# tyb311/TCCT

Measured on AMD Instinct MI355X. Metric: OCT B-scans/sec fwd+bwd(+clip+AdamW), stc_tt bs=8 1x800x1100, higher is better.
Workload: dtype bf16; 1 GPU; stc_tt --los=di bs=8/GPU 1x800x1100 (net tensors 3x800x1104); global_batch=8, parallelism=dp1, ranks=1, grad_allreduce=none, slowest_step=66

## Files before the change

include/tcct_hip.h:

```cpp
#ifndef TCCT_HIP_H
#define TCCT_HIP_H
#include <stdint.h>
#ifdef __cplusplus
extern "C" {
#endif

typedef void* tcct_stream_t;

enum { TCCT_F32 = 0, TCCT_BF16 = 1 };
enum { TCCT_ACT_NONE = 0, TCCT_ACT_LRELU = 1, TCCT_ACT_HSWISH = 2, TCCT_ACT_GELU = 3, TCCT_ACT_SIGMOID = 4,
       TCCT_ACT_ABS = 5 };
enum { TCCT_CRIT_DICE = 0, TCCT_CRIT_DICE2 = 1, TCCT_CRIT_IOU = 2, TCCT_CRIT_MSE = 3 };

int tcct_version(void);
const char* tcct_last_error(void);
int tcct_set_outputs_prezeroed(int on);

int tcct_image_to_nhwc4(const float* img, void* out, int N, int Csrc, int H, int Wsrc, int Wdst, int dtype,
                        tcct_stream_t stream);
int tcct_u8_gather2d(const uint8_t* src, uint8_t* dst, int N, int SH, int SW, int C, int sy0, int sx0, int sh, int sw, int DH, int DW,
                     int dy0, int dx0, int dh, int dw, int flipy, int flipx, int mul, int div, int fill, tcct_stream_t stream);
int tcct_onehot_to_index(const int64_t* onehot, uint8_t* lab, int N, int C, int64_t HW, tcct_stream_t stream);
int tcct_labels_to_u8(const int64_t* lab, uint8_t* out, int N, int H, int Wsrc, int Wdst, tcct_stream_t stream);
int tcct_nhwc_to_nchw_f32(const void* x, float* y, int N, int64_t HW, int C, int dtype, tcct_stream_t stream);
// ... 97 lines not shown

int tcct_conv32_fwd_bnstats(const void* x, const void* wp, const float* bias, void* y, int N, int H, int W, int KH, int KW, int PH,
                            int PW, double* stats, int pre_act, tcct_stream_t stream);
int tcct_conv32_fwd_affine(const void* x, const void* wp, const float* bias, void* y, int N, int H, int W, int KH, int KW,
                           int PH, int PW, const float* ab, int pre_act, int post_act, tcct_stream_t stream);
int tcct_pw_fwd_affine(const void* x, const float* w, const float* bias, void* y, int64_t M, int K, int N, const float* ab,
                       int pre_act, int post_act, int out_dtype, tcct_stream_t stream);
int tcct_pw_fwd_affine_residual(const void* x, const float* w, const float* bias, const float* ab, const void* res, void* y, int64_t M, int K, int N,
                                tcct_stream_t stream);
int tcct_pw_fwd_cat2_affine(const void* x1, const void* x2, const float* w, const float* bias, const float* ab, int post_act, void* y, int64_t M, int K, int N,
                            tcct_stream_t stream);
int tcct_pw_fwd_xaff_affine_residual(const void* y_prev, const float* ab_prev, const float* w, const float* bias, const float* ab, const void* res, void* y,
                                     int64_t M, int K, int N, tcct_stream_t stream);
int tcct_conv32_fwd_add(const void* x, const void* wp, const float* bias, const void* res, void* y, int N, int H, int W, int KH, int KW,
                        int PH, int PW, tcct_stream_t stream);
int tcct_conv32_chain33(const void* x, const void* wp1, const float* bias1, void* mid, const void* wp2, const float* bias2, void* y,
                        const void* res, int N, int H, int W, double* stats, tcct_stream_t stream);
int tcct_conv32_pack_weights_sub(const float* w, void* wp, int KH, int KW, int transposed, int cin_total, int o_off, int i_off,
                                 tcct_stream_t stream);
int tcct_conv32_fwd_strided(const void* x, const void* wp, const float* bias, void* y, int N, int H, int W, int KH, int KW, int PH,
                            int PW, int xs, int xo, int ys, int yo, int accumulate, tcct_stream_t stream);
int tcct_conv32_fwd_strided_bnstats(const void* x, const void* wp, const float* bias, void* y, int N, int H, int W, int KH, int KW, int PH,
                                    int PW, int xs, int xo, int ys, int yo, int accumulate, double* stats, int pre_act, tcct_stream_t stream);
int tcct_conv32_fwd_strided_affine(const void* x, const void* wp, const float* bias, void* y, int N, int H, int W, int KH, int KW, int PH, int PW, int xs,
                                   int xo, int ys, int yo, const float* ab, int pre_act, int post_act, tcct_stream_t stream);
int64_t tcct_conv32_wgrad_mode(int mode);
int64_t tcct_conv32_fwd_mode(int mode);
int tcct_conv32_wgrad_strided(const void* x, const void* dy, float* dw, float* dbias, int N, int H, int W, int KH, int KW, int PH,
                              int PW, int xs, int xo, int ds, int dof, int cin_total, int o_off, int i_off, tcct_stream_t stream);
int tcct_conv32_wgrad(const void* x, const void* dy, float* dw, float* dbias, int N, int H, int W, int KH, int KW, int PH,
                      int PW, tcct_stream_t stream);
int tcct_conv32_bwd3x3(const void* x, const void* dy, const void* wp_t, const void* dskip, void* dx, float* dw, float* dbias, int N, int H,
                       int W, tcct_stream_t stream);

int tcct_pw_fwd(const void* x, const float* w, const float* bias, void* y, int64_t M, int K, int N, int transposed,
                int out_dtype, tcct_stream_t stream);
int tcct_pw_wgrad(const void* x, const void* dy, float* dw, float* dbias, int64_t M, int K, int N, tcct_stream_t stream);
int tcct_pw_bwd(const void* x, const void* dy, const float* w, const void* res, void* dx, float* dw, float* dbias, int64_t M, int K, int N,
                tcct_stream_t stream);
int tcct_pw_bwd_cat2(const void* x1, const void* x2, const void* dy, const float* w, void* dx1, void* dx2, float* dw, int64_t M, int K, int N,
                     tcct_stream_t stream);
int tcct_pw_bwd_residual2(const void* x, const void* dy, const float* w, const void* res, void* dx_sum, void* dx_plain, float* dw, float* dbias,
                          int64_t M, int K, int N, tcct_stream_t stream);
int64_t tcct_pw_bwd_bn_supported(int K, int N, int post, int red_post, int split);
int tcct_pw_bwd_bn(const void* x, const void* x2, const void* dz, const void* y, const float* coef, int post, const float* w, const void* res,
                   void* dx, void* dx2, float* dw, float* dbias, int64_t M, int K, int N, const void* y_prev, const float* ab_prev,
                   int red_post, double* sums_prev, tcct_stream_t stream);
int tcct_pw_bwd_bn_sums(const void* x, const void* x2, const void* dz, const void* y, const double* sums, int raw, const float* mean_rstd,
                        const float* ab, float* dgamma, float* dbeta, int post, const float* w, const void* res, void* dx, void* dx2, float* dw,
                        float* dbias, int64_t M, int K, int N, const void* y_prev, const float* ab_prev, int red_post, double* sums_prev,
                        tcct_stream_t stream);
int tcct_pw_wgrad_strided(const void* x, const void* dy, int64_t ldy, float* dw, float* dbias, int64_t M, int K, int N,
                          tcct_stream_t stream);
int tcct_pw_fwd_residual(const void* x, const float* w, const float* bias, const void* res, const float* scale, int64_t per_sample,
                         void* y, void* y_plain, int64_t M, int K, int N, tcct_stream_t stream);
int tcct_pw_fwd_bnstats_xaff(const void* y_prev, const float* ab_prev, const float* w, const float* bias, void* y, int64_t M, int K, int N, double* stats,
                             tcct_stream_t stream);
int tcct_pw_bwd_bn_sums_xaff(const void* y_prev, const float* ab_prev, const void* dz, const void* y, const double* sums, int raw, const float* mean_rstd,
                             const float* ab, float* dgamma, float* dbeta, const float* w, const void* res, void* dx, float* dw, float* dbias, int64_t M,
                             int K, int N, int red_post, double* sums_prev, tcct_stream_t stream);
int tcct_pw_fwd_gelu_residual(const void* x1, const float* w, const float* bias, const void* res, const float* scale, int64_t per_sample, void* y,
                              int64_t M, int K, int N, tcct_stream_t stream);
int tcct_pw_bwd_residual2_sum(const void* x, const void* dy_a, const void* dy_b, const float* w, const void* res, void* dx_sum, void* dx_plain, float* dw,
                              float* dbias, int64_t M, int K, int N, tcct_stream_t stream);
int tcct_pw_bwd_lnb(const void* x, const void* dy, const float* w, const void* t, const float* mean_rstd, const float* gamma, const void* res, void* dt,
                    float* dw, float* dbias, float* dgamma, float* dbeta, int64_t M, int K, int N, tcct_stream_t stream);
// ... 203 lines not shown
```

tcct_amd/csrc/conv_mfma.hip:

```cpp
#include "common.h"

typedef __attribute__((ext_vector_type(8))) __bf16 bf16x8;
typedef __attribute__((ext_vector_type(16))) float f32x16;

#define MB 256
#define OOB_OFF 0x80000000u

__global__ void k_pack_w32(const float* __restrict__ w, bf16* __restrict__ wp, int KH, int KW, int transposed, int ldi,
                           int o_off, int i_off) {
    int total = KH * KW * 32 * 32;
    for (int i = blockIdx.x * blockDim.x + threadIdx.x; i < total; i += gridDim.x * blockDim.x) {
        int ci = i & 31, co = (i >> 5) & 31, tap = i >> 10;
        int dy = tap / KW, dx = tap % KW;
        const float vt = w[(((int64_t)(o_off + ci) * ldi + i_off + co) * KH + (KH - 1 - dy)) * KW + (KW - 1 - dx)];
        const float vn = w[(((int64_t)(o_off + co) * ldi + i_off + ci) * KH + dy) * KW + dx];
        if (transposed == 2) { wp[i] = __float2bfloat16(vn); wp[total + i] = __float2bfloat16(vt); }
        else wp[i] = __float2bfloat16(transposed ? vt : vn);
    }
}
extern "C" int tcct_conv32_pack_weights(const float* w, void* wp, int KH, int KW, int transposed, tcct_stream_t stream) {
    int total = KH * KW * 1024;
    hipLaunchKernelGGL(k_pack_w32, dim3((total + MB - 1) / MB), dim3(MB), 0, (hipStream_t)stream, w, (bf16*)wp, KH, KW, transposed, 32, 0, 0);
    TCCT_LAUNCH_OK();
}
// ... 1812 lines not shown
            TCCT_LAUNCH_OK();
        }
    }
    constexpr bool line_on = true;
    if (line_on && g_wgrad_mode != 1 && (KH == 1 || KW == 1) && (TAPS == 13 || TAPS == 11 || TAPS == 9) && xs == 32 && ds == 32 && ldi == 32 && o_off == 0 && i_off == 0 &&
        xo == 0 && dof == 0) {
#define WL_LAUNCH(KK, V)                                                                                                     \
    do {                                                                                                                    \
        tcct_launch<k_conv32_wgrad_line<KK, V>, 80 * 1024>(dim3(grid), dim3(MB), (size_t)(8 * (64 + KK - 1) + 16) * 64 + 512 * 64, st, (const bf16*)x, (const bf16*)dy, \
                           dw, dbias, N, H, W, tilesH, tilesW, (int)nt);                                                    \
    } while (0)
        if (TAPS == 13) { if (vert) WL_LAUNCH(13, true); else WL_LAUNCH(13, false); }
        else if (TAPS == 11) { if (vert) WL_LAUNCH(11, true); else WL_LAUNCH(11, false); }
        else { if (vert) WL_LAUNCH(9, true); else WL_LAUNCH(9, false); }
#undef WL_LAUNCH
        TCCT_LAUNCH_OK();
    }
    const int TG = TAPS > 10 ? 4 : (TAPS > 5 ? 2 : 1);
    const int tpw = (TAPS + TG - 1) / TG;
    TCCT_CHECK(TAPS <= 16, "conv32_wgrad: %d taps unsupported", TAPS);
    TCCT_CHECK(LH * LW * 4 <= MAXL * MB, "conv32_wgrad: %dx%d tile image exceeds the staging slots", KH, KW);
#define WG_LAUNCH(TPW, V, Q)                                                                                                 \
    do {                                                                                                                    \
        tcct_launch<k_conv32_wgrad<TPW, V, Q>, 80 * 1024>(dim3(grid), dim3(MB), lds, st, (const bf16*)x, (const bf16*)dy, dw, dbias, N, H, W, KH, \
                           KW, PH, PW, TG, tilesH, tilesW, (int)nt, xs, xo, ds, dof, ldi, o_off, i_off);                                                        \
    } while (0)
    if (sq) WG_LAUNCH(5, false, true);
    else if (tpw <= 4) { if (vert) WG_LAUNCH(4, true, false); else WG_LAUNCH(4, false, false); }
    else { if (vert) WG_LAUNCH(5, true, false); else WG_LAUNCH(5, false, false); }
#undef WG_LAUNCH
    TCCT_LAUNCH_OK();
}

#define BWD_T 512
template <int DUMMY>
__global__ void __launch_bounds__(BWD_T, 1)
k_conv32_bwd33(const bf16* __restrict__ x, const bf16* __restrict__ dy, const bf16* __restrict__ wp, const bf16* __restrict__ dskip,
               bf16* __restrict__ dx, float* __restrict__ dw, float* __restrict__ dbias, int N, int H, int W, int tilesH, int tilesW,
               int ntiles) {
    constexpr int TH = 16, TW = 32, LH = 18, LW = 34, NPIX = LH * LW, SLOTS = (NPIX * 4 + BWD_T - 1) / BWD_T;
    extern __shared__ __attribute__((aligned(16))) unsigned char smem[];
    unsigned char* sW = smem;
    unsigned char* sXl = smem + 9 * 2048;
    unsigned char* sDp = sXl + NPIX * 64;
    unsigned char* sS = sDp + NPIX * IPS;
    const int tid = threadIdx.x, lane = tid & 63, wave = tid >> 6;
    const int r = lane & 31, hh = lane >> 5;
    for (int i = tid; i < 9 * 32 * 4; i += BWD_T) {
        int row = i >> 2, c4 = i & 3;
        uint4 v = reinterpret_cast<const uint4*>(wp)[i];
        *reinterpret_cast<uint4*>(sW + row * 64 + ((c4 ^ ((row >> 2) & 3)) << 4)) = v;
    }
    const int c = tid & 3;
    int s_rc[SLOTS];
#pragma unroll
    for (int j = 0; j < SLOTS; ++j) {
        int pl = (tid >> 2) + j * (BWD_T / 4);
        bool in = pl < NPIX;
        int lr = in ? pl / LW : 0x3fff, lc = in ? pl - (pl / LW) * LW : 0;
        s_rc[j] = (lr << 16) | lc;
    }
    const uint32_t img_bytes = (uint32_t)H * (uint32_t)W * 64u;
    u32x4 px[SLOTS], pd[SLOTS];
    auto prefetch = [&](int tile) {
        const int tw = tile % tilesW;
        const int t2 = tile / tilesW;
        const int th = t2 % tilesH;
        const int n = t2 / tilesH;
        const int hb = th * TH - 1, wb = tw * TW - 1;
        const __amdgpu_buffer_rsrc_t rx = __builtin_amdgcn_make_buffer_rsrc((void*)(x + (int64_t)n * H * W * 32), 0, img_bytes, 0x00020000);
        const __amdgpu_buffer_rsrc_t rd = __builtin_amdgcn_make_buffer_rsrc((void*)(dy + (int64_t)n * H * W * 32), 0, img_bytes, 0x00020000);
#pragma unroll
        for (int j = 0; j < SLOTS; ++j) {
            const int hi = hb + (s_rc[j] >> 16), wi = wb + (s_rc[j] & 0xffff);
            const bool ok = (unsigned)hi < (unsigned)H && (unsigned)wi < (unsigned)W;
            const uint32_t off = ok ? (uint32_t)((hi * W + wi) * 64 + c * 16) : OOB_OFF;
            px[j] = __builtin_amdgcn_raw_buffer_load_b128(rx, off, 0, 0);
            pd[j] = __builtin_amdgcn_raw_buffer_load_b128(rd, off, 0, 0);
        }
    };
    auto stage = [&]() {
#pragma unroll
        for (int j = 0; j < SLOTS; ++j) {
            const int lr = s_rc[j] >> 16, lc = s_rc[j] & 0xffff;
            if (lr != 0x3fff) {
                const int p = lr * LW + lc;
                *reinterpret_cast<u32x4*>(sXl + p * 64 + c * 16) = px[j];
                *reinterpret_cast<u32x4*>(sDp + p * IPS + c * 16) = pd[j];
            }
        }
    };
    const int wsw = (r >> 2) & 3;
    const unsigned char* wA0 = sW + r * 64 + ((hh ^ wsw) << 4);
    const unsigned char* wA1 = sW + r * 64 + (((2 + hh) ^ wsw) << 4);
    const int dwave = wave & 3;
    const unsigned char* xB[4];
#pragma unroll
    for (int t = 0; t < 4; ++t) xB[t] = sDp + ((dwave * 4 + t) * LW + r) * IPS + hh * 16;
    const int tg = (wave >> 1) & 1, wi = wave & 1;
    const int tap0 = tg * 5;
    int poff[5];
#pragma unroll
    for (int t = 0; t < 5; ++t) {
        const int tap = tap0 + t, ky = tap / 3, kx = tap - ky * 3;
        poff[t] = tap < 9 ? (ky * LW + kx) * 64 : 0;
    }
    f32x16 accw[5];
#pragma unroll
    for (int t = 0; t < 5; ++t)
#pragma unroll
        for (int k = 0; k < 16; ++k) accw[t][k] = 0.f;
    float bsum = 0.f;
    const int li = lane & 15, lq = li >> 2, lpp = li & 3, lg = lane >> 4;
    const unsigned char* lbX = sXl + (8 * (lg >> 1) + lq) * 64 + (16 * (lg & 1) + 4 * lpp) * 2;
    const unsigned char* lbD = sDp + (8 * (lg >> 1) + lq) * IPS + (16 * (lg & 1) + 4 * lpp) * 2;
    auto tr8 = [&](const unsigned char* p, int stride) {
        s16x4 lo = __builtin_amdgcn_ds_read_tr16_b64_v4i16((__attribute__((address_space(3))) s16x4*)p);
        s16x4 hi = __builtin_amdgcn_ds_read_tr16_b64_v4i16((__attribute__((address_space(3))) s16x4*)(p + 4 * stride));
        s16x8 v = __builtin_shufflevector(lo, hi, 0, 1, 2, 3, 4, 5, 6, 7);
        return __builtin_bit_cast(bf16x8, v);
    };

    int tile = blockIdx.x;
    if (tile < ntiles) {
        prefetch(tile);
        __syncthreads();
        stage();
        if (tile + (int)gridDim.x < ntiles) prefetch(tile + gridDim.x);
    }
    __syncthreads();
    for (; tile < ntiles; tile += gridDim.x) {
        const int tw = tile % tilesW;
        const int t2 = tile / tilesW;
        const int th = t2 % tilesH;
        const int n = t2 / tilesH;
        const int h0 = th * TH, w0 = tw * TW;
        f32x16* const acc = accw;
        if (wave < 4) {
#pragma unroll
            for (int t = 0; t < 4; ++t)
#pragma unroll
                for (int k = 0; k < 16; ++k) acc[t][k] = 0.f;
            struct Frag { bf16x8 a, b[4]; };
            auto load_stage = [&](Frag& f, int ky, int kx, int half) {
                f.a = *reinterpret_cast<const bf16x8*>((half ? wA1 : wA0) + (ky * 3 + kx) * 2048);
                const int po = (ky * LW + kx) * IPS + half * 32;
#pragma unroll
                for (int t = 0; t < 4; ++t) f.b[t] = *reinterpret_cast<const bf16x8*>(xB[t] + po);
            };
            Frag f[2];
            load_stage(f[0], 0, 0, 0);
#pragma unroll
            for (int k = 0; k < 18; ++k) {
                if (k + 1 < 18) load_stage(f[(k + 1) & 1], ((k + 1) >> 1) / 3, ((k + 1) >> 1) % 3, (k + 1) & 1);
                __builtin_amdgcn_sched_barrier(0);
#pragma unroll
                for (int t = 0; t < 4; ++t) acc[t] = __builtin_amdgcn_mfma_f32_32x32x16_bf16(f[k & 1].a, f[k & 1].b[t], acc[t], 0, 0, 0);
                __builtin_amdgcn_sched_barrier(0);
            }
        } else {
            struct WF { bf16x8 a, b[5]; };
            auto load_chunk = [&](WF& f, int ch) {
                const int a = ch >> 1, s16 = (ch & 1) * 16;
                f.a = tr8(lbD + ((a + 1) * LW + s16 + 1) * IPS, IPS);
                const unsigned char* pxb = lbX + (a * LW + s16) * 64;
#pragma unroll
                for (int t = 0; t < 5; ++t) f.b[t] = tr8(pxb + poff[t], 64);
            };
            auto mma_chunk = [&](const WF& f) {
                if (tg == 0) {
#pragma unroll
                    for (int j = 0; j < 4; ++j) bsum = dot2_ones(f.a, j, bsum);
                }
#pragma unroll
                for (int t = 0; t < 5; ++t)
                    if (tap0 + t < 9) accw[t] = __builtin_amdgcn_mfma_f32_32x32x16_bf16(f.a, f.b[t], accw[t], 0, 0, 0);
            };
            WF f0, f1;
            load_chunk(f0, wi);
            for (int ch = wi; ch < 32; ch += 4) {
                load_chunk(f1, ch + 2);
                __builtin_amdgcn_sched_barrier(0);
                mma_chunk(f0);
                __builtin_amdgcn_sched_barrier(0);
                if (ch + 4 < 32) load_chunk(f0, ch + 4);
                __builtin_amdgcn_sched_barrier(0);
                mma_chunk(f1);
                __builtin_amdgcn_sched_barrier(0);
            }
        }
        __syncthreads();
        if (tile + (int)gridDim.x < ntiles) stage();
        if (tile + 2 * (int)gridDim.x < ntiles) prefetch(tile + 2 * gridDim.x);
        if (wave < 4) {
            const __amdgpu_buffer_rsrc_t ws = __builtin_amdgcn_make_buffer_rsrc((void*)(dx + (int64_t)n * H * W * 32), 0, img_bytes, 0x00020000);
            const __amdgpu_buffer_rsrc_t rsk = __builtin_amdgcn_make_buffer_rsrc((void*)((dskip ? dskip : dx) + (int64_t)n * H * W * 32), 0, img_bytes, 0x00020000);
            unsigned char* sc = sS + dwave * 1024;
#pragma unroll
            for (int t = 0; t < 4; ++t) {
                const int a = dwave * 4 + t;
                uint2 o[4];
#pragma unroll
                for (int q = 0; q < 4; ++q) {
                    o[q].x = pack_bf16x2(acc[t][4 * q], acc[t][4 * q + 1]);
                    o[q].y = pack_bf16x2(acc[t][4 * q + 2], acc[t][4 * q + 3]);
                }
#pragma unroll
                for (int h2 = 0; h2 < 2; ++h2) {
                    if ((r >> 4) == h2) {
                        const int rr = r & 15, fsw = (rr >> 1) & 3;
#pragma unroll
                        for (int q = 0; q < 4; ++q) *reinterpret_cast<uint2*>(sc + rr * 64 + ((q ^ fsw) << 4) + hh * 8) = o[q];
                    }
                    wave_lds_fence();
                    const int p16 = lane >> 2, cch = lane & 3;
                    u32x4 ov = *reinterpret_cast<const u32x4*>(sc + p16 * 64 + ((cch ^ ((p16 >> 1) & 3)) << 4));
                    const int ho = h0 + a, wo = w0 + 16 * h2 + p16;
                    const uint32_t off = (ho < H && wo < W) ? (uint32_t)((ho * W + wo) * 64 + cch * 16) : OOB_OFF;
                    if (dskip) {
                        const u32x4 sv = __builtin_amdgcn_raw_buffer_load_b128(rsk, off, 0, 0);
#pragma unroll
                        for (int k = 0; k < 4; ++k)
                            ov[k] = pack_bf16x2(__uint_as_float(ov[k] << 16) + __uint_as_float(sv[k] << 16),
                                                __uint_as_float(ov[k] & 0xffff0000u) + __uint_as_float(sv[k] & 0xffff0000u));
                    }
                    __builtin_amdgcn_raw_buffer_store_b128(ov, ws, off, 0, 0);
                    wave_lds_fence();
                }
            }
        }
        __syncthreads();
    }
    __syncthreads();
    float* red = reinterpret_cast<float*>(sXl);
    for (int turn = 0; turn < 2; ++turn) {
        if (wave >= 4 && wi == turn) {
#pragma unroll
            for (int t = 0; t < 5; ++t) {
                const int tap = tap0 + t;
                if (tap < 9) {
#pragma unroll
                    for (int k = 0; k < 16; ++k) {
                        const int co = (k & 3) + 8 * (k >> 2) + 4 * hh;
                        float* dst = &red[tap * 1024 + co * 32 + r];
                        *dst = turn == 0 ? accw[t][k] : *dst + accw[t][k];
                    }
                }
            }
        }
        __syncthreads();
    }
    for (int i = tid; i < 9 * 1024; i += BWD_T) {
        const int tap = i % 9, cc = i / 9;
        atomicAdd(&dw[(int64_t)cc * 9 + tap], red[tap * 1024 + cc]);
    }
    if (dbias && wave >= 4 && tg == 0) {
        bsum += __shfl_xor(bsum, 32, 64);
        if (lane < 32) atomicAdd(&dbias[r], bsum);
    }
}

extern "C" int tcct_conv32_bwd3x3(const void* x, const void* dy, const void* wp_t, const void* dskip, void* dx, float* dw, float* dbias,
                                  int N, int H, int W, tcct_stream_t stream) {
    TCCT_CHECK((int64_t)H * W * 64 < (1LL << 31), "conv32_bwd3x3: image exceeds the 2 GiB buffer-descriptor range");
    TCCT_CHECK(dskip != dx, "conv32_bwd3x3: dskip must be a separate tensor");
    hipStream_t st = (hipStream_t)stream;
    if (!tcct_skip_zero_fill() && hipMemsetAsync(dw, 0, sizeof(float) * 9 * 1024, st) != hipSuccess) { tcct_set_error("conv32_bwd3x3: memset failed"); return -2; }
    if (dbias && !tcct_skip_zero_fill() && hipMemsetAsync(dbias, 0, sizeof(float) * 32, st) != hipSuccess) { tcct_set_error("conv32_bwd3x3: memset failed"); return -2; }
    const int tilesH = (H + 15) / 16, tilesW = (W + 31) / 32;
    const int64_t nt = (int64_t)N * tilesH * tilesW;
    TCCT_CHECK(nt > 0 && nt < (1LL << 31), "conv32_bwd3x3: bad tile count");
    const size_t lds = 9 * 2048 + (size_t)18 * 34 * 64 + (size_t)18 * 34 * IPS + 4096;
    const int grid = (int)(nt < 256 ? nt : 256);
    tcct_launch<k_conv32_bwd33<0>, 160 * 1024>(dim3(grid), dim3(BWD_T), lds, st, (const bf16*)x, (const bf16*)dy, (const bf16*)wp_t, (const bf16*)dskip,
                       (bf16*)dx, dw, dbias, N, H, W, tilesH, tilesW, (int)nt);
    TCCT_LAUNCH_OK();
}
```

tcct_amd/ops.py:

```python
import os
import weakref

import torch

from ._lib import lib, dtype_code, TcctError, launch_on, F32, BF16

ACT = {None: 0, 'none': 0, 'lrelu': 1, 'hswish': 2, 'gelu': 3, 'sigmoid': 4, 'abs': 5}


class _ZeroPool:

    def __init__(self):
        self.buf = None
        self.off = 0
        self.active = False
        self.frozen = False

    def begin(self, device, nbytes=8 << 20):
        if self.buf is None or self.buf.device != device or self.buf.numel() < nbytes:
            if self.frozen:
                raise TcctError('the zero pool cannot be re-allocated after a training step was captured into a hipGraph '
                                f'(pool on {self.buf.device}, step on {device})')
            self.buf = torch.empty(nbytes, device=device, dtype=torch.uint8)
        self.buf.zero_()
# ... 277 lines not shown
            and 32 <= Cin <= 256 and 32 <= Cout <= 256 and (Cin, Cout) != (32, 32) and stride == 1
            and 2 * padh == KH - 1 and 2 * padw == KW - 1 and 1 < KH * KW <= 13 and (KH == 1 or KW == 1 or (KH == 3 and KW == 3)))


def _conv_slabs_fwd_f32(x, w, bias, y, N, H, W, Cin, Cout, KH, KW, padh, padw, transposed):
    for oh in range(Cout // 32):
        for ih in range(Cin // 32):
            wp = torch.empty(KH * KW * 1024, device=x.device, dtype=torch.float32)
            if not transposed:
                lib.conv32f_pack_weights_sub(w, wp, KH, KW, 0, Cin, 32 * oh, 32 * ih)
            else:
                lib.conv32f_pack_weights_sub(w, wp, KH, KW, 1, Cout, 32 * ih, 32 * oh)
            b = bias[32 * oh:32 * oh + 32] if (bias is not None and ih == 0) else None
            lib.conv32f_fwd_strided(x, wp, b, y, N, H, W, KH, KW, padh, padw, Cin, 32 * ih, Cout, 32 * oh, 1 if ih > 0 else 0)


def _conv_slabs_fwd(x, w, bias, y, N, H, W, Cin, Cout, KH, KW, padh, padw, transposed, stats=None, stat_pre=0):
    wp = torch.empty(KH * KW * 1024, device=x.device, dtype=torch.bfloat16)
    for oh in range(Cout // 32):
        for ih in range(Cin // 32):
            if not transposed:
                lib.conv32_pack_weights_sub(w, wp, KH, KW, 0, Cin, 32 * oh, 32 * ih)
            else:
                lib.conv32_pack_weights_sub(w, wp, KH, KW, 1, Cout, 32 * ih, 32 * oh)
            b = bias[32 * oh:32 * oh + 32] if (bias is not None and ih == 0) else None
            if stats is not None and ih == Cin // 32 - 1:
                lib.conv32_fwd_strided_bnstats(x, wp, b, y, N, H, W, KH, KW, padh, padw, Cin, 32 * ih, Cout, 32 * oh, 1 if ih > 0 else 0, stats, stat_pre)
            else:
                lib.conv32_fwd_strided(x, wp, b, y, N, H, W, KH, KW, padh, padw, Cin, 32 * ih, Cout, 32 * oh, 1 if ih > 0 else 0)
            if ih + 1 < Cin // 32 or oh + 1 < Cout // 32:
                wp = torch.empty_like(wp)


FUSED_CONV_BWD = False
FUSED_PW_BWD = True


def _pw_bwd_ok(x, dy, Cin, Cin_w, Cout, KH, KW, stride, padh, padw):
    return (x.dtype == torch.bfloat16 and dy.dtype == torch.bfloat16 and KH == 1 and KW == 1 and stride == 1 and padh == 0 and padw == 0
            and Cin == Cin_w and Cin % 32 == 0 and Cout % 32 == 0 and 32 <= Cin <= 128 and 32 <= Cout <= 128
            and x.numel() * 2 < 2 ** 31 and dy.numel() * 2 < 2 ** 31)


def _pw_ok(in_dt, Cin, Cin_w, KH, KW, stride, padh, padw):
    return (in_dt == torch.bfloat16 and KH == 1 and KW == 1 and stride == 1 and padh == 0 and padw == 0 and Cin == Cin_w
            and Cin % 32 == 0)


class _Conv2d(_FastFunction):
    @staticmethod
    def forward(ctx, x, w, bias, stride, padh, padw, out_dtype, stats_box, fork=False):
        ctx.set_materialize_grads(False)
        _chk(x, w, bias)
        N, H, W, Cin = x.shape
        Cout, Cin_w, KH, KW = w.shape
        Ho = (H + 2 * padh - KH) // stride + 1
        Wo = (W + 2 * padw - KW) // stride + 1
        odt = out_dtype or x.dtype
        y = torch.empty((N, Ho, Wo, Cout), device=x.device, dtype=odt)
        mfma = _mfma32_ok(x.dtype, odt, Cin, Cin_w, Cout, KH, KW, stride, padh, padw)
        if _pw_ok(x.dtype, Cin, Cin_w, KH, KW, stride, padh, padw) and not mfma:
            if stats_box is not None and odt == torch.bfloat16 and Cout % 32 == 0 and Cout <= 160:
                sums = ZERO.get((2 * Cout,), torch.float64, x.device) if ZERO.active else torch.zeros(2 * Cout, device=x.device, dtype=torch.float64)
                lib.pw_fwd_bnstats(x, w, bias, y, N * H * W, Cin, Cout, sums, stats_box[0])
                stats_box[1] = sums
            else:
                lib.pw_fwd(x, w, bias, y, N * H * W, Cin, Cout, 0, dtype_code(odt))
# ... 28 lines not shown
            _conv_slabs_fwd_f32(x, w, bias, y, N, H, W, Cin, Cout, KH, KW, padh, padw, False)
        elif F32_PW[0] and _pwf_ok(x.dtype, odt, Cin, Cin_w, Cout, KH, KW, stride, padh, padw):
            lib.pwf_fwd(x, w, bias, y, N * H * W, Cin, Cout, 0)
        else:
            lib.conv2d_fwd(x, w, bias, y, N, H, W, Cin, Cin_w, Cout, KH, KW, stride, padh, padw, dtype_code(x.dtype),
                           dtype_code(odt))
        ctx.save_for_backward(x, w)
        ctx.cfg = (stride, padh, padw, bias is not None)
        wsrc = w if hasattr(w, '_grad_slot') or w._base is None else w._base
        ctx.params = (wsrc, bias)
        return (y, x.view_as(x)) if fork else y

    @staticmethod
    def backward(ctx, dy, dskip=None):
        x, w = ctx.saved_tensors
        stride, padh, padw, has_bias = ctx.cfg
        wsrc, bsrc = ctx.params
        if dy is None:
            return dskip, None, None, None, None, None, None, None, None
        dy = _c(dy)
        if dskip is not None:
            dskip = _as(dskip, x.dtype)
        N, H, W, Cin = x.shape
        Cout, Cin_w, KH, KW = w.shape
        dx = dw = db = None
        if (FUSED_PW_BWD and ctx.needs_input_grad[0] and ctx.needs_input_grad[1] and _pw_bwd_ok(x, dy, Cin, Cin_w, Cout, KH, KW, stride, padh, padw)
                and (dskip is None or dskip.shape == x.shape)):
            dx = torch.empty_like(x)
            dw = _grad_out(wsrc, tuple(w.shape))
            db = _grad_out(bsrc) if has_bias else None
            lib.pw_bwd(x, dy, w, dskip, dx, dw, db, N * H * W, Cin, Cout)
            return dx, _ret(dw, wsrc), _ret(db, bsrc), None, None, None, None, None, None
        if (FUSED_CONV_BWD and ctx.needs_input_grad[0] and ctx.needs_input_grad[1] and KH == 3 and KW == 3 and dy.dtype == torch.bfloat16
                and _mfma32_ok(x.dtype, dy.dtype, Cin, Cin_w, Cout, KH, KW, stride, padh, padw) and H * W * 64 < 2 ** 31):
            wp = getattr(ctx, 'wp_t', None)
            if wp is None:
                wp = torch.empty(9 * 1024, device=x.device, dtype=torch.bfloat16)
                lib.conv32_pack_weights(w, wp, 3, 3, 1)
            dx = torch.empty_like(x)
            dw = _grad_out(wsrc, tuple(w.shape))
            db = _grad_out(bsrc) if has_bias else None
            lib.conv32_bwd3x3(x, dy, wp, dskip, dx, dw, db, N, H, W)
            return dx, _ret(dw, wsrc), _ret(db, bsrc), None, None, None, None, None, None
        if ctx.needs_input_grad[0]:
            if stride != 1 or Cin != Cin_w:
                raise TcctError('conv2d dgrad: only stride-1 convs with unpadded channels need an input gradient')
            dx = torch.empty_like(x)
            if (_pw_ok(dy.dtype, Cout, Cout, KH, KW, stride, padh, padw) and x.dtype == torch.bfloat16
                    and not _mfma32_ok(dy.dtype, x.dtype, Cout, Cout, Cin, KH, KW, stride, padh, padw)):
                if dskip is not None and Cin % 32 == 0:
                    lib.pw_dgrad_residual(dy, w, dskip, dx, None, N * H * W, Cout, Cin)
                    dskip = None
                else:
                    lib.pw_fwd(dy, w, None, dx, N * H * W, Cout, Cin, 1, dtype_code(x.dtype))
            elif _mfma_slabs_ok(dy.dtype, x.dtype, Cout, Cout, Cin, KH, KW, stride, padh, padw):
                _conv_slabs_fwd(dy, w, None, dx, N, H, W, Cout, Cin, KH, KW, KH - 1 - padh, KW - 1 - padw, True)
            elif _mfma32_ok(dy.dtype, x.dtype, Cout, Cout, Cin, KH, KW, stride, padh, padw):
                wp = getattr(ctx, 'wp_t', None)
                if wp is None:
                    wp = torch.empty(KH * KW * 1024, device=x.device, dtype=torch.bfloat16)
                    lib.conv32_pack_weights(w, wp, KH, KW, 1)
                if dskip is not None:
                    lib.conv32_fwd_add(dy, wp, None, dskip, dx, N, H, W, KH, KW, KH - 1 - padh, KW - 1 - padw)
                    dskip = None
                else:
                    lib.conv32_fwd(dy, wp, None, dx, N, H, W, KH, KW, KH - 1 - padh, KW - 1 - padw)
            elif _mfma_slabs_f32_ok(dy.dtype, x.dtype, Cout, Cout, Cin, KH, KW, stride, padh, padw):
# ... 2785 lines not shown
```

Measured before the change: 420.5 B-scans/s.

## Stream fused 3x3 conv backward over row strips with LDS DMA ring and enable it

```diff
diff --git a/include/tcct_hip.h b/include/tcct_hip.h
--- a/include/tcct_hip.h
+++ b/include/tcct_hip.h
@@ -153,6 +153,8 @@
                       int PW, tcct_stream_t stream);
 int tcct_conv32_bwd3x3(const void* x, const void* dy, const void* wp_t, const void* dskip, void* dx, float* dw, float* dbias, int N, int H,
                        int W, tcct_stream_t stream);
+int64_t tcct_conv32_bwd_mode(int mode);
+int64_t tcct_conv32_bwd_streams(int N, int H, int W);
 
 int tcct_pw_fwd(const void* x, const float* w, const float* bias, void* y, int64_t M, int K, int N, int transposed,
                 int out_dtype, tcct_stream_t stream);
diff --git a/tcct_amd/csrc/conv_mfma.hip b/tcct_amd/csrc/conv_mfma.hip
--- a/tcct_amd/csrc/conv_mfma.hip
+++ b/tcct_amd/csrc/conv_mfma.hip
@@ -1868,247 +1868,294 @@
     TCCT_LAUNCH_OK();
 }
 
-#define BWD_T 512
-template <int DUMMY>
-__global__ void __launch_bounds__(BWD_T, 1)
-k_conv32_bwd33(const bf16* __restrict__ x, const bf16* __restrict__ dy, const bf16* __restrict__ wp, const bf16* __restrict__ dskip,
-               bf16* __restrict__ dx, float* __restrict__ dw, float* __restrict__ dbias, int N, int H, int W, int tilesH, int tilesW,
-               int ntiles) {
-    constexpr int TH = 16, TW = 32, LH = 18, LW = 34, NPIX = LH * LW, SLOTS = (NPIX * 4 + BWD_T - 1) / BWD_T;
+#define BS_T 256
+#ifndef BS_R
+#define BS_R 6
+#endif
+#ifndef BS_P
+#define BS_P 4
+#endif
+#define BS_MIN_RUN 48
+static_assert(BS_R % 3 == 0 && BS_P <= BS_R - 2 && BS_P >= 1, "k_conv32_bwd33_stream: ring geometry");
+template <bool SKIP>
+__global__ void __launch_bounds__(BS_T, 1)
+k_conv32_bwd33_stream(const bf16* __restrict__ x, const bf16* __restrict__ dy, const bf16* __restrict__ wp, const bf16* __restrict__ dskip,
+                      bf16* __restrict__ dx, float* __restrict__ dw, float* __restrict__ dbias, int N, int H, int W, int strips, int run, int rpi) {
+    constexpr int XOFF = 2176, SOFF = 4352;
+    constexpr int ROWB = SKIP ? 6400 : 4352;
+    constexpr int NPIECE = SKIP ? 8 : 6;
+    static_assert(NPIECE * (BS_P - 1) < 64, "vmcnt is a 6-bit counter");
     extern __shared__ __attribute__((aligned(16))) unsigned char smem[];
-    unsigned char* sW = smem;
-    unsigned char* sXl = smem + 9 * 2048;
-    unsigned char* sDp = sXl + NPIX * 64;
-    unsigned char* sS = sDp + NPIX * IPS;
-    const int tid = threadIdx.x, lane = tid & 63, wave = tid >> 6;
+    const int tid = threadIdx.x, lane = tid & 63, wave = __builtin_amdgcn_readfirstlane(tid >> 6);
     const int r = lane & 31, hh = lane >> 5;
-    for (int i = tid; i < 9 * 32 * 4; i += BWD_T) {
-        int row = i >> 2, c4 = i & 3;
-        uint4 v = reinterpret_cast<const uint4*>(wp)[i];
-        *reinterpret_cast<uint4*>(sW + row * 64 + ((c4 ^ ((row >> 2) & 3)) << 4)) = v;
-    }
-    const int c = tid & 3;
-    int s_rc[SLOTS];
-#pragma unroll
-    for (int j = 0; j < SLOTS; ++j) {
-        int pl = (tid >> 2) + j * (BWD_T / 4);
-        bool in = pl < NPIX;
-        int lr = in ? pl / LW : 0x3fff, lc = in ? pl - (pl / LW) * LW : 0;
-        s_rc[j] = (lr << 16) | lc;
-    }
-    const uint32_t img_bytes = (uint32_t)H * (uint32_t)W * 64u;
-    u32x4 px[SLOTS], pd[SLOTS];
-    auto prefetch = [&](int tile) {
-        const int tw = tile % tilesW;
-        const int t2 = tile / tilesW;
-        const int th = t2 % tilesH;
-        const int n = t2 / tilesH;
-        const int hb = th * TH - 1, wb = tw * TW - 1;
-        const __amdgpu_buffer_rsrc_t rx = __builtin_amdgcn_make_buffer_rsrc((void*)(x + (int64_t)n * H * W * 32), 0, img_bytes, 0x00020000);
-        const __amdgpu_buffer_rsrc_t rd = __builtin_amdgcn_make_buffer_rsrc((void*)(dy + (int64_t)n * H * W * 32), 0, img_bytes, 0x00020000);
-#pragma unroll
-        for (int j = 0; j < SLOTS; ++j) {
-            const int hi = hb + (s_rc[j] >> 16), wi = wb + (s_rc[j] & 0xffff);
-            const bool ok = (unsigned)hi < (unsigned)H && (unsigned)wi < (unsigned)W;
-            const uint32_t off = ok ? (uint32_t)((hi * W + wi) * 64 + c * 16) : OOB_OFF;
-            px[j] = __builtin_amdgcn_raw_buffer_load_b128(rx, off, 0, 0);
-            pd[j] = __builtin_amdgcn_raw_buffer_load_b128(rd, off, 0, 0);
-        }
-    };
-    auto stage = [&]() {
-#pragma unroll
-        for (int j = 0; j < SLOTS; ++j) {
-            const int lr = s_rc[j] >> 16, lc = s_rc[j] & 0xffff;
-            if (lr != 0x3fff) {
-                const int p = lr * LW + lc;
-                *reinterpret_cast<u32x4*>(sXl + p * 64 + c * 16) = px[j];
-                *reinterpret_cast<u32x4*>(sDp + p * IPS + c * 16) = pd[j];
-            }
-        }
-    };
-    const int wsw = (r >> 2) & 3;
-    const unsigned char* wA0 = sW + r * 64 + ((hh ^ wsw) << 4);
-    const unsigned char* wA1 = sW + r * 64 + (((2 + hh) ^ wsw) << 4);
-    const int dwave = wave & 3;
-    const unsigned char* xB[4];
-#pragma unroll
-    for (int t = 0; t < 4; ++t) xB[t] = sDp + ((dwave * 4 + t) * LW + r) * IPS + hh * 16;
-    const int tg = (wave >> 1) & 1, wi = wave & 1;
-    const int tap0 = tg * 5;
-    int poff[5];
-#pragma unroll
-    for (int t = 0; t < 5; ++t) {
-        const int tap = tap0 + t, ky = tap / 3, kx = tap - ky * 3;
-        poff[t] = tap < 9 ? (ky * LW + kx) * 64 : 0;
-    }
-    f32x16 accw[5];
-#pragma unroll
-    for (int t = 0; t < 5; ++t)
-#pragma unroll
-        for (int k = 0; k < 16; ++k) accw[t][k] = 0.f;
-    float bsum = 0.f;
-    const int li = lane & 15, lq = li >> 2, lpp = li & 3, lg = lane >> 4;
-    const unsigned char* lbX = sXl + (8 * (lg >> 1) + lq) * 64 + (16 * (lg & 1) + 4 * lpp) * 2;
-    const unsigned char* lbD = sDp + (8 * (lg >> 1) + lq) * IPS + (16 * (lg & 1) + 4 * lpp) * 2;
-    auto tr8 = [&](const unsigned char* p, int stride) {
-        s16x4 lo = __builtin_amdgcn_ds_read_tr16_b64_v4i16((__attribute__((address_space(3))) s16x4*)p);
-        s16x4 hi = __builtin_amdgcn_ds_read_tr16_b64_v4i16((__attribute__((address_space(3))) s16x4*)(p + 4 * stride));
+    unsigned char* ring = smem + wave * (BS_R * ROWB);
+    const uint32_t ring_lds = __builtin_amdgcn_readfirstlane((uint32_t)(size_t)(__attribute__((address_space(3))) unsigned char*)ring);
+    bf16x8 Wf[9][2];
+#pragma unroll
+    for (int t = 0; t < 9; ++t)
+#pragma unroll
+        for (int kc = 0; kc < 2; ++kc) Wf[t][kc] = *reinterpret_cast<const bf16x8*>(wp + (t * 32 + r) * 32 + (hh + 2 * kc) * 8);
+    const unsigned char* xB[3][2];
+#pragma unroll
+    for (int d = 0; d < 3; ++d)
+#pragma unroll
+        for (int kc = 0; kc < 2; ++kc) { const int P = r + d; xB[d][kc] = ring + P * 64 + (((hh + 2 * kc) ^ ((P >> 2) & 3)) << 4); }
+    const unsigned char* xT = tr_lane_base(ring + XOFF, lane);
+    const unsigned char* dT[2][2];
+    {
+        const int i = lane & 15, q = i >> 2, pp = i & 3, g = lane >> 4;
+        const int ch = 2 * (g & 1) + (pp >> 1);
+#pragma unroll
+        for (int k = 0; k < 2; ++k)
+#pragma unroll
+            for (int h2 = 0; h2 < 2; ++h2) {
+                const int P = 1 + 16 * k + 8 * (g >> 1) + q + 4 * h2;
+                dT[k][h2] = ring + P * 64 + ((ch ^ ((P >> 2) & 3)) << 4) + 8 * (pp & 1);
+            }
+    }
+    auto tr2 = [](const unsigned char* lo_p, const unsigned char* hi_p) {
+        s16x4 lo = __builtin_amdgcn_ds_read_tr16_b64_v4i16((__attribute__((address_space(3))) s16x4*)lo_p);
+        s16x4 hi = __builtin_amdgcn_ds_read_tr16_b64_v4i16((__attribute__((address_space(3))) s16x4*)hi_p);
         s16x8 v = __builtin_shufflevector(lo, hi, 0, 1, 2, 3, 4, 5, 6, 7);
         return __builtin_bit_cast(bf16x8, v);
     };
-
-    int tile = blockIdx.x;
-    if (tile < ntiles) {
-        prefetch(tile);
-        __syncthreads();
-        stage();
-        if (tile + (int)gridDim.x < ntiles) prefetch(tile + gridDim.x);
-    }
+    f32x16 accw[9];
+#pragma unroll
+    for (int t = 0; t < 9; ++t)
+#pragma unroll
+        for (int k = 0; k < 16; ++k) accw[t][k] = 0.f;
+    float bsum = 0.f;
+    const int sgroups = (strips + 3) >> 2;
+    const int bq = blockIdx.x / sgroups, grp = blockIdx.x - bq * sgroups;
+    const int n = bq / rpi, r0 = (bq - n * rpi) * run;
+    const int L = __builtin_amdgcn_readfirstlane(H - r0 < run ? H - r0 : run);
+    const int s = grp * 4 + wave;
+    const int groups = (L + 2 + BS_R - 1) / BS_R;
+    const uint32_t img_bytes = (uint32_t)H * (uint32_t)W * 64u;
+    const uint32_t rowb = (uint32_t)W * 64u;
+    if (s < strips) {
+        const int pq = lane >> 2, c = lane & 3, cs = c ^ ((lane >> 4) & 3);
+        const int w0 = s * 32;
+        const u32x4 rdy = make_rsrc_words(dy + (int64_t)n * H * W * 32, img_bytes);
+        const u32x4 rxx = make_rsrc_words(x + (int64_t)n * H * W * 32, img_bytes);
+        const u32x4 rsk = make_rsrc_words((SKIP ? dskip : dy) + (int64_t)n * H * W * 32, img_bytes);
+        const __amdgpu_buffer_rsrc_t ws = __builtin_amdgcn_make_buffer_rsrc((void*)(dx + (int64_t)n * H * W * 32), 0, img_bytes, 0x00020000);
+        const int c0 = w0 - 1 + pq, c1 = w0 + 15 + pq, c2 = w0 + 31 + pq;
+        const bool in0 = c0 >= 0 && c0 < W, in1 = c1 < W, in2 = c2 < W;
+        const uint32_t od0 = in0 ? (uint32_t)(c0 * 64 + cs * 16) : OOB_OFF, od1 = in1 ? (uint32_t)(c1 * 64 + cs * 16) : OOB_OFF,
+                       od2 = in2 ? (uint32_t)(c2 * 64 + cs * 16) : OOB_OFF;
+        const uint32_t ox0 = in0 ? (uint32_t)(c0 * 64 + c * 16) : OOB_OFF, ox1 = in1 ? (uint32_t)(c1 * 64 + c * 16) : OOB_OFF,
+                       ox2 = in2 ? (uint32_t)(c2 * 64 + c * 16) : OOB_OFF;
+        const int k0 = w0 + pq, k1 = w0 + 16 + pq;
+        const uint32_t os0 = k0 < W ? (uint32_t)(k0 * 64 + cs * 16) : OOB_OFF, os1 = k1 < W ? (uint32_t)(k1 * 64 + cs * 16) : OOB_OFF;
+        const int p16 = lane >> 2, cch = lane & 3;
+        uint32_t so[2];
+#pragma unroll
+        for (int u = 0; u < 2; ++u) { const int wo = w0 + 16 * u + p16; so[u] = wo < W ? (uint32_t)(wo * 64 + cch * 16) : OOB_OFF; }
+        const uint32_t row0 = (uint32_t)(r0 - 1) * rowb;
+        auto issue = [&](int a, int slot) {
+            const uint32_t ro = row0 + (uint32_t)a * rowb;
+            const bool in = a <= L + 1;
+            const uint32_t base = ring_lds + (uint32_t)(slot * ROWB);
+            lds_dma16(rdy, in ? od0 + ro : OOB_OFF, base);
+            lds_dma16(rdy, in ? od1 + ro : OOB_OFF, base + 1024u);
+            if (lane < 8) lds_dma16(rdy, in ? od2 + ro : OOB_OFF, base + 2048u);
+            lds_dma16(rxx, in ? ox0 + ro : OOB_OFF, base + (uint32_t)XOFF);
+            lds_dma16(rxx, in ? ox1 + ro : OOB_OFF, base + (uint32_t)XOFF + 1024u);
+            if (lane < 8) lds_dma16(rxx, in ? ox2 + ro : OOB_OFF, base + (uint32_t)XOFF + 2048u);
+            if (SKIP) {
+                lds_dma16(rsk, in ? os0 + ro : OOB_OFF, base + (uint32_t)SOFF);
+                lds_dma16(rsk, in ? os1 + ro : OOB_OFF, base + (uint32_t)SOFF + 1024u);
+            }
+        };
+#pragma unroll
+        for (int a = 0; a < BS_P; ++a) issue(a, a);
+        asm volatile("s_waitcnt vmcnt(%0)" :: "n"(NPIECE * (BS_P - 1)) : "memory");
+        bf16x8 Xd[3][2], Xdn[3][2], Xt[3][2], Xtn[3][2], Dw[3][2], Dn[2];
+#pragma unroll
+        for (int d = 0; d < 3; ++d)
+#pragma unroll
+            for (int kc = 0; kc < 2; ++kc) {
+                Xd[d][kc] = *reinterpret_cast<const bf16x8*>(xB[d][kc]);
+                Xt[d][kc] = tr_load8p(xT + (d + 16 * kc) * 64);
+            }
+        bf16x8 zero8;
+#pragma unroll
+        for (int k = 0; k < 8; ++k) zero8[k] = (__bf16)0.f;
+#pragma unroll
+        for (int t = 0; t < 3; ++t) { Dw[t][0] = zero8; Dw[t][1] = zero8; }
+        f32x16 acc[3];
+        for (int g = 0; g < groups; ++g) {
+            __builtin_amdgcn_s_barrier();
+#pragma unroll
+            for (int j = 0; j < BS_R; ++j) {
+                const int a = g * BS_R + j;
+                issue(a + BS_P, (j + BS_P) % BS_R);
+                asm volatile("s_waitcnt vmcnt(%0)" :: "n"(NPIECE * (BS_P - 1)) : "memory");
+                const int nso = ((j + 1) % BS_R) * ROWB;
+#pragma unroll
+                for (int k = 0; k < 2; ++k) Dn[k] = tr2(dT[k][0] + nso, dT[k][1] + nso);
+#pragma unroll
+                for (int d = 0; d < 3; ++d)
+#pragma unroll
+                    for (int kc = 0; kc < 2; ++kc) Xdn[d][kc] = *reinterpret_cast<const bf16x8*>(xB[d][kc] + nso);
+#pragma unroll
+                for (int d = 0; d < 3; ++d)
+#pragma unroll
+                    for (int kc = 0; kc < 2; ++kc) Xtn[d][kc] = tr_load8p(xT + nso + (d + 16 * kc) * 64);
+#pragma unroll
+                for (int k = 0; k < 16; ++k) acc[j % 3][k] = 0.f;
+                __builtin_amdgcn_sched_barrier(0);
+#pragma unroll
+                for (int ty = 0; ty < 3; ++ty)
+#pragma unroll
+                    for (int d = 0; d < 3; ++d)
+#pragma unroll
+                        for (int kc = 0; kc < 2; ++kc)
+                            acc[(j + 3 - ty) % 3] = __builtin_amdgcn_mfma_f32_32x32x16_bf16(Wf[ty * 3 + d][kc], Xd[d][kc], acc[(j + 3 - ty) % 3], 0, 0, 0);
+#pragma unroll
+                for (int q = 0; q < 4; ++q) { bsum = dot2_ones(Dw[j % 3][0], q, bsum); bsum = dot2_ones(Dw[j % 3][1], q, bsum); }
+                const bool dv = a + 1 <= L;
+                Dw[(j + 1) % 3][0] = dv ? Dn[0] : zero8;
+                Dw[(j + 1) % 3][1] = dv ? Dn[1] : zero8;
+#pragma unroll
+                for (int ty = 2; ty >= 0; --ty)
+#pragma unroll
+                    for (int d = 0; d < 3; ++d)
+#pragma unroll
+                        for (int kc = 0; kc < 2; ++kc)
+                            accw[ty * 3 + d] = __builtin_amdgcn_mfma_f32_32x32x16_bf16(Dw[(j + 4 - ty) % 3][kc], Xt[d][kc], accw[ty * 3 + d], 0, 0, 0);
+                __builtin_amdgcn_sched_barrier(0);
+                const int orow = a - 2;
+                const bool ovalid = orow >= 0 && orow < L;
+                f32x16& A = acc[(j + 1) % 3];
+                unsigned char* sc = ring + ((j + BS_R - 1) % BS_R) * ROWB;
+                uint2 o[4];
+#pragma unroll
+                for (int q = 0; q < 4; ++q) {
+                    float v4[4] = {A[4 * q], A[4 * q + 1], A[4 * q + 2], A[4 * q + 3]};
+                    if constexpr (SKIP) {
+                        const uint2 sv = *reinterpret_cast<const uint2*>(sc + SOFF + r * 64 + ((q ^ ((r >> 2) & 3)) << 4) + hh * 8);
+                        v4[0] += __uint_as_float(sv.x << 16); v4[1] += __uint_as_float(sv.x & 0xffff0000u);
+                        v4[2] += __uint_as_float(sv.y << 16); v4[3] += __uint_as_float(sv.y & 0xffff0000u);
+                    }
+                    o[q].x = pack_bf16x2(v4[0], v4[1]); o[q].y = pack_bf16x2(v4[2], v4[3]);
+                }
+                const int f = (r >> 1) & 3;
+#pragma unroll
+                for (int q = 0; q < 4; ++q) *reinterpret_cast<uint2*>(sc + r * 64 + ((q ^ f) << 4) + hh * 8) = o[q];
+                wave_lds_fence();
+                u32x4 pend[2];
+#pragma unroll
+                for (int u = 0; u < 2; ++u) pend[u] = *reinterpret_cast<const u32x4*>(sc + (16 * u + p16) * 64 + ((cch ^ ((p16 >> 1) & 3)) << 4));
+                wave_lds_fence();
+                const uint32_t oro = (uint32_t)(r0 + orow) * rowb;
+#pragma unroll
+                for (int u = 0; u < 2; ++u) {
+                    const bool inb = ovalid && so[u] != OOB_OFF;
+                    __builtin_amdgcn_raw_buffer_store_b128(pend[u], ws, inb ? so[u] + oro : OOB_OFF, 0, 0);
+                }
+                __builtin_amdgcn_sched_barrier(0);
+#pragma unroll
+                for (int d = 0; d < 3; ++d)
+#pragma unroll
+                    for (int kc = 0; kc < 2; ++kc) { Xd[d][kc] = Xdn[d][kc]; Xt[d][kc] = Xtn[d][kc]; }
+            }
+        }
+    } else {
+        for (int g = 0; g < groups; ++g) __builtin_amdgcn_s_barrier();
+    }
+    asm volatile("s_waitcnt vmcnt(0)" ::: "memory");
     __syncthreads();
-    for (; tile < ntiles; tile += gridDim.x) {
-        const int tw = tile % tilesW;
-        const int t2 = tile / tilesW;
-        const int th = t2 % tilesH;
-        const int n = t2 / tilesH;
-        const int h0 = th * TH, w0 = tw * TW;
-        f32x16* const acc = accw;
-        if (wave < 4) {
-#pragma unroll
-            for (int t = 0; t < 4; ++t)
-#pragma unroll
-                for (int k = 0; k < 16; ++k) acc[t][k] = 0.f;
-            struct Frag { bf16x8 a, b[4]; };
-            auto load_stage = [&](Frag& f, int ky, int kx, int half) {
-                f.a = *reinterpret_cast<const bf16x8*>((half ? wA1 : wA0) + (ky * 3 + kx) * 2048);
-                const int po = (ky * LW + kx) * IPS + half * 32;
-#pragma unroll
-                for (int t = 0; t < 4; ++t) f.b[t] = *reinterpret_cast<const bf16x8*>(xB[t] + po);
-            };
-            Frag f[2];
-            load_stage(f[0], 0, 0, 0);
-#pragma unroll
-            for (int k = 0; k < 18; ++k) {
-                if (k + 1 < 18) load_stage(f[(k + 1) & 1], ((k + 1) >> 1) / 3, ((k + 1) >> 1) % 3, (k + 1) & 1);
-                __builtin_amdgcn_sched_barrier(0);
-#pragma unroll
-                for (int t = 0; t < 4; ++t) acc[t] = __builtin_amdgcn_mfma_f32_32x32x16_bf16(f[k & 1].a, f[k & 1].b[t], acc[t], 0, 0, 0);
-                __builtin_amdgcn_sched_barrier(0);
-            }
-        } else {
-            struct WF { bf16x8 a, b[5]; };
-            auto load_chunk = [&](WF& f, int ch) {
-                const int a = ch >> 1, s16 = (ch & 1) * 16;
-                f.a = tr8(lbD + ((a + 1) * LW + s16 + 1) * IPS, IPS);
-                const unsigned char* pxb = lbX + (a * LW + s16) * 64;
-#pragma unroll
-                for (int t = 0; t < 5; ++t) f.b[t] = tr8(pxb + poff[t], 64);
-            };
-            auto mma_chunk = [&](const WF& f) {
-                if (tg == 0) {
-#pragma unroll
-                    for (int j = 0; j < 4; ++j) bsum = dot2_ones(f.a, j, bsum);
-                }
-#pragma unroll
-                for (int t = 0; t < 5; ++t)
-                    if (tap0 + t < 9) accw[t] = __builtin_amdgcn_mfma_f32_32x32x16_bf16(f.a, f.b[t], accw[t], 0, 0, 0);
-            };
-            WF f0, f1;
-            load_chunk(f0, wi);
-            for (int ch = wi; ch < 32; ch += 4) {
-                load_chunk(f1, ch + 2);
-                __builtin_amdgcn_sched_barrier(0);
-                mma_chunk(f0);
-                __builtin_amdgcn_sched_barrier(0);
-                if (ch + 4 < 32) load_chunk(f0, ch + 4);
-                __builtin_amdgcn_sched_barrier(0);
-                mma_chunk(f1);
-                __builtin_amdgcn_sched_barrier(0);
-            }
-        }
-        __syncthreads();
-        if (tile + (int)gridDim.x < ntiles) stage();
-        if (tile + 2 * (int)gridDim.x < ntiles) prefetch(tile + 2 * gridDim.x);
-        if (wave < 4) {
-            const __amdgpu_buffer_rsrc_t ws = __builtin_amdgcn_make_buffer_rsrc((void*)(dx + (int64_t)n * H * W * 32), 0, img_bytes, 0x00020000);
-            const __amdgpu_buffer_rsrc_t rsk = __builtin_amdgcn_make_buffer_rsrc((void*)((dskip ? dskip : dx) + (int64_t)n * H * W * 32), 0, img_bytes, 0x00020000);
-            unsigned char* sc = sS + dwave * 1024;
-#pragma unroll
-            for (int t = 0; t < 4; ++t) {
-                const int a = dwave * 4 + t;
-                uint2 o[4];
-#pragma unroll
-                for (int q = 0; q < 4; ++q) {
-                    o[q].x = pack_bf16x2(acc[t][4 * q], acc[t][4 * q + 1]);
-                    o[q].y = pack_bf16x2(acc[t][4 * q + 2], acc[t][4 * q + 3]);
-                }
-#pragma unroll
-                for (int h2 = 0; h2 < 2; ++h2) {
-                    if ((r >> 4) == h2) {
-                        const int rr = r & 15, fsw = (rr >> 1) & 3;
-#pragma unroll
-                        for (int q = 0; q < 4; ++q) *reinterpret_cast<uint2*>(sc + rr * 64 + ((q ^ fsw) << 4) + hh * 8) = o[q];
-                    }
-                    wave_lds_fence();
-                    const int p16 = lane >> 2, cch = lane & 3;
-                    u32x4 ov = *reinterpret_cast<const u32x4*>(sc + p16 * 64 + ((cch ^ ((p16 >> 1) & 3)) << 4));
-                    const int ho = h0 + a, wo = w0 + 16 * h2 + p16;
-                    const uint32_t off = (ho < H && wo < W) ? (uint32_t)((ho * W + wo) * 64 + cch * 16) : OOB_OFF;
-                    if (dskip) {
-                        const u32x4 sv = __builtin_amdgcn_raw_buffer_load_b128(rsk, off, 0, 0);
-#pragma unroll
-                        for (int k = 0; k < 4; ++k)
-                            ov[k] = pack_bf16x2(__uint_as_float(ov[k] << 16) + __uint_as_float(sv[k] << 16),
-                                                __uint_as_float(ov[k] & 0xffff0000u) + __uint_as_float(sv[k] & 0xffff0000u));
-                    }
-                    __builtin_amdgcn_raw_buffer_store_b128(ov, ws, off, 0, 0);
-                    wave_lds_fence();
-                }
-            }
-        }
-        __syncthreads();
-    }
-    __syncthreads();
-    float* red = reinterpret_cast<float*>(sXl);
-    for (int turn = 0; turn < 2; ++turn) {
-        if (wave >= 4 && wi == turn) {
-#pragma unroll
-            for (int t = 0; t < 5; ++t) {
-                const int tap = tap0 + t;
-                if (tap < 9) {
-#pragma unroll
-                    for (int k = 0; k < 16; ++k) {
-                        const int co = (k & 3) + 8 * (k >> 2) + 4 * hh;
-                        float* dst = &red[tap * 1024 + co * 32 + r];
-                        *dst = turn == 0 ? accw[t][k] : *dst + accw[t][k];
-                    }
-                }
-            }
-        }
-        __syncthreads();
-    }
-    for (int i = tid; i < 9 * 1024; i += BWD_T) {
+    float* red = reinterpret_cast<float*>(smem);
+    for (int turn = 0; turn < BS_T / 64; ++turn) {
+        if (wave == turn) {
+#pragma unroll
+            for (int t = 0; t < 9; ++t)
+#pragma unroll
+                for (int k = 0; k < 16; ++k) {
+                    const int co = (k & 3) + 8 * (k >> 2) + 4 * hh;
+                    float* dst = &red[t * 1024 + co * 32 + r];
+                    *dst = turn == 0 ? accw[t][k] : *dst + accw[t][k];
+                }
+        }
+        __syncthreads();
+    }
+    for (int i = tid; i < 9 * 1024; i += BS_T) {
         const int tap = i % 9, cc = i / 9;
         atomicAdd(&dw[(int64_t)cc * 9 + tap], red[tap * 1024 + cc]);
     }
-    if (dbias && wave >= 4 && tg == 0) {
+    __syncthreads();
+    if (dbias) {
         bsum += __shfl_xor(bsum, 32, 64);
-        if (lane < 32) atomicAdd(&dbias[r], bsum);
-    }
+        if (lane < 32) red[wave * 32 + r] = bsum;
+        __syncthreads();
+        if (tid < 32) atomicAdd(&dbias[tid], red[tid] + red[32 + tid] + red[64 + tid] + red[96 + tid]);
+    }
+}
+
+static int g_bwd_mode = -1;
+extern "C" int64_t tcct_conv32_bwd_mode(int mode) {
+    if (g_bwd_mode < 0) g_bwd_mode = 0;
+    const int prev = g_bwd_mode;
+    if (mode >= 0 && mode <= 2) g_bwd_mode = mode;
+    return prev;
+}
+static bool conv32_bwd_plan(int N, int H, int W, int* run_o, int* rpi_o, int* blocks_o) {
+    if (g_bwd_mode < 0) (void)tcct_conv32_bwd_mode(-1);
+    if (g_bwd_mode == 1 || N < 1 || H < 1 || W < 1 || ((int64_t)H + 2) * W * 64 >= (1LL << 31)) return false;
+    const int strips = (W + 31) / 32, sg = (strips + 3) / 4;
+    const bool force = g_bwd_mode == 2;
+    int maxr = H / (force ? 12 : BS_MIN_RUN);
+    if (maxr > 16 && !force) maxr = 16;
+    if (maxr < 1) { if (!force) return false; maxr = 1; }
+    int rpi = maxr;
+    if (!force) {
+        double best = -1.0;
+        for (int c = 1; c <= maxr; ++c) {
+            const int64_t b = (int64_t)N * sg * c;
+            const double eff = (double)b / (double)(((b + 255) / 256) * 256);
+            if (eff > best + 1e-9) { best = eff; rpi = c; }
+        }
+    }
+    const int run = (H + rpi - 1) / rpi;
+    rpi = (H + run - 1) / run;
+    const int64_t blocks = (int64_t)N * rpi * sg;
+    if (blocks >= (1LL << 31) || (!force && blocks < 192)) return false;
+    *run_o = run; *rpi_o = rpi; *blocks_o = (int)blocks;
+    return true;
+}
+extern "C" int64_t tcct_conv32_bwd_streams(int N, int H, int W) {
+    int run, rpi, blocks;
+    return conv32_bwd_plan(N, H, W, &run, &rpi, &blocks) ? 1 : 0;
 }
 
 extern "C" int tcct_conv32_bwd3x3(const void* x, const void* dy, const void* wp_t, const void* dskip, void* dx, float* dw, float* dbias,
                                   int N, int H, int W, tcct_stream_t stream) {
     TCCT_CHECK((int64_t)H * W * 64 < (1LL << 31), "conv32_bwd3x3: image exceeds the 2 GiB buffer-descriptor range");
     TCCT_CHECK(dskip != dx, "conv32_bwd3x3: dskip must be a separate tensor");
+    int run, rpi, blocks;
+    if (!conv32_bwd_plan(N, H, W, &run, &rpi, &blocks)) {
+        const int rc = conv32_fwd_impl(dy, wp_t, nullptr, dx, N, H, W, 3, 3, 1, 1, 32, 0, 32, 0, dskip ? 1 : 0, nullptr, 0, stream, nullptr, 0, false, dskip);
+        if (rc != 0) return rc;
+        return conv32_wgrad_impl(x, dy, dw, dbias, N, H, W, 3, 3, 1, 1, 32, 0, 32, 0, 32, 0, 0, 1, stream);
+    }
     hipStream_t st = (hipStream_t)stream;
     if (!tcct_skip_zero_fill() && hipMemsetAsync(dw, 0, sizeof(float) * 9 * 1024, st) != hipSuccess) { tcct_set_error("conv32_bwd3x3: memset failed"); return -2; }
     if (dbias && !tcct_skip_zero_fill() && hipMemsetAsync(dbias, 0, sizeof(float) * 32, st) != hipSuccess) { tcct_set_error("conv32_bwd3x3: memset failed"); return -2; }
-    const int tilesH = (H + 15) / 16, tilesW = (W + 31) / 32;
-    const int64_t nt = (int64_t)N * tilesH * tilesW;
-    TCCT_CHECK(nt > 0 && nt < (1LL << 31), "conv32_bwd3x3: bad tile count");
-    const size_t lds = 9 * 2048 + (size_t)18 * 34 * 64 + (size_t)18 * 34 * IPS + 4096;
-    const int grid = (int)(nt < 256 ? nt : 256);
-    tcct_launch<k_conv32_bwd33<0>, 160 * 1024>(dim3(grid), dim3(BWD_T), lds, st, (const bf16*)x, (const bf16*)dy, (const bf16*)wp_t, (const bf16*)dskip,
-                       (bf16*)dx, dw, dbias, N, H, W, tilesH, tilesW, (int)nt);
+    const int strips = (W + 31) / 32;
+    if (dskip) {
+        constexpr size_t lds = (size_t)(BS_T / 64) * BS_R * 6400;
+        static_assert(lds <= 160 * 1024 && lds >= 9 * 4096, "k_conv32_bwd33_stream<true>: ring size");
+        tcct_launch<k_conv32_bwd33_stream<true>, 160 * 1024>(dim3((unsigned)blocks), dim3(BS_T), lds, st, (const bf16*)x, (const bf16*)dy, (const bf16*)wp_t,
+                                                              (const bf16*)dskip, (bf16*)dx, dw, dbias, N, H, W, strips, run, rpi);
+    } else {
+        constexpr size_t lds = (size_t)(BS_T / 64) * BS_R * 4352;
+        static_assert(lds <= 160 * 1024 && lds >= 9 * 4096, "k_conv32_bwd33_stream<false>: ring size");
+        tcct_launch<k_conv32_bwd33_stream<false>, 160 * 1024>(dim3((unsigned)blocks), dim3(BS_T), lds, st, (const bf16*)x, (const bf16*)dy, (const bf16*)wp_t,
+                                                               (const bf16*)dskip, (bf16*)dx, dw, dbias, N, H, W, strips, run, rpi);
+    }
+    tcct_census_hit(TCCT_CENSUS_FWD33_STREAM);
+    tcct_census_hit(TCCT_CENSUS_WGRAD33_STREAM);
     TCCT_LAUNCH_OK();
 }
diff --git a/tcct_amd/ops.py b/tcct_amd/ops.py
--- a/tcct_amd/ops.py
+++ b/tcct_amd/ops.py
@@ -333,7 +333,7 @@
                 wp = torch.empty_like(wp)
 
 
-FUSED_CONV_BWD = False
+FUSED_CONV_BWD = True
 FUSED_PW_BWD = True
 
 
@@ -428,7 +428,8 @@
             lib.pw_bwd(x, dy, w, dskip, dx, dw, db, N * H * W, Cin, Cout)
             return dx, _ret(dw, wsrc), _ret(db, bsrc), None, None, None, None, None, None
         if (FUSED_CONV_BWD and ctx.needs_input_grad[0] and ctx.needs_input_grad[1] and KH == 3 and KW == 3 and dy.dtype == torch.bfloat16
-                and _mfma32_ok(x.dtype, dy.dtype, Cin, Cin_w, Cout, KH, KW, stride, padh, padw) and H * W * 64 < 2 ** 31):
+                and _mfma32_ok(x.dtype, dy.dtype, Cin, Cin_w, Cout, KH, KW, stride, padh, padw) and H * W * 64 < 2 ** 31
+                and (dskip is None or dskip.shape == x.shape) and lib.conv32_bwd_streams(N, H, W)):
             wp = getattr(ctx, 'wp_t', None)
             if wp is None:
                 wp = torch.empty(9 * 1024, device=x.device, dtype=torch.bfloat16)
```

Result: no change. 422.2 B-scans/s (median of 6 runs) (+0.4%).
